# jhamrick/bayesian-quadrature

Measured on AMD Instinct MI355X. Metric: bq_fit_posterior_throughput, higher is better.
Workload: dtype f64; 1 GPU; C2: d=1 N=1024 M=256 Gaussian integrand, w=dx, s=1e-3; curve_workload=C5 shard: 64 x (d=1 N=2048 M=256), w=dx, s=1e-2, on_curve=True, bordered_system=1344

## Files before the change

bayesian-quadrature_amd/_lib.py:

```python
import ctypes as C
import os

import numpy as np

_HERE = os.path.dirname(os.path.abspath(__file__))
LIB_PATH = os.environ.get("BQHIP_LIBRARY") or os.path.join(_HERE, "libbqhip.so")
PROBE_LIB_PATH = os.environ.get("BQHIP_PROBE_LIBRARY") or \
    os.path.splitext(LIB_PATH)[0] + "_probe.so"

BQ_OK, BQ_ERR_NOT_PD, BQ_ERR_BAD_ARG, BQ_ERR_HIP, BQ_ERR_NOMEM = 0, 1, 2, 3, 4
BQ_MAX_DIM = 8
K_CLASSES = ("gram", "potf2", "trsm", "gemm_panel", "syrk_trailing", "syrk_trailing_small",
             "reduce")

_dp = C.POINTER(C.c_double)
_i32p = C.POINTER(C.c_int32)
_i64p = C.POINTER(C.c_int64)
_vp = C.c_void_p
_i64 = C.c_int64
_dbl = C.c_double

SIGNATURES = {
    "bq_device_count": (C.c_int, [C.POINTER(C.c_int)]),
    "bq_ctx_create": (C.c_int, [C.c_int, C.POINTER(_vp)]),
# ... 76 lines not shown
PROBE_SIGNATURES = {
    "bq_probe_xcd_hop": (C.c_int, [_vp, C.c_int, C.c_int64, C.c_int64, C.POINTER(C.c_double), _i32p,
                                   C.POINTER(C.c_int64)]),
    "bq_probe_mfma_f64": (C.c_int, [_vp, _dp]),
    "bq_probe_fma_f64": (C.c_int, [_vp, _dp]),
    "bq_probe_hbm": (C.c_int, [_vp, C.c_size_t, _dp, _dp]),
    "bq_probe_hbm_read8": (C.c_int, [_vp, C.c_size_t, _i64, _dp]),
    "bq_probe_gemm": (C.c_int, [_vp, _i64, _i64, _i64, C.c_int, _i64, C.c_int, _i64, _dp]),
    "bq_probe_gemm_product": (C.c_int, [_vp, _dp, _i64, _dp, _i64, _dp, _i64, _i64, _i64, _i64,
                                        C.c_int, _i64, C.c_int, _i64, C.c_int, C.c_int, _i64, C.c_int,
                                        C.c_int, _dp, _i32p, _i32p]),
    "bq_probe_mfma_variant": (C.c_int, [_vp, C.c_int, C.c_int, C.c_int, _dp]),
    "bq_probe_mfma444_layout": (C.c_int, [_vp, C.c_int, C.c_int, _i32p]),
    "bq_probe_launch": (C.c_int, [_vp, _i64, _dp]),
    "bq_probe_c2_timeline": (C.c_int, [_vp, _vp, C.POINTER(C.c_int64), _i64]),
    "bq_probe_exp": (C.c_int, [_vp, _dp, _i64, _dp]),
    "bq_probe_potf2": (C.c_int, [_vp, _dp, C.c_int, _i64, _dp, _dp, C.POINTER(C.c_int32), _dp,
                                 C.POINTER(C.c_int64)]),
    "bq_probe_mfma_layout": (C.c_int, [_vp, _dp]),
    "bq_probe_panel_solve": (C.c_int, [_vp, _i64, _i64, _i64, _dp, _dp, C.c_int, _i64, _dp]),
    "bq_probe_potrf_batch": (C.c_int, [_vp, _i64, _i64, _i64, _i64, _i64, _dp, _i32p, _i32p]),
    "bq_probe_sweep": (C.c_int, [_vp, C.c_int, _i64, _dp, _i64, _i64, _i64, _dp, _i32p]),
}

_lib = None
_probe_lib = None


class LibraryMissing(ImportError):
    pass
# ... 46 lines not shown
```

bayesian-quadrature_amd/csrc/ctx.hip:

```cpp
#include "host.h"

namespace bqh {

int prof_collect(bq_ctx *c)
{
    if (c->prof_events.empty())
        return BQ_OK;
    HIPCHK(c, hipStreamSynchronize(c->stream));
    if (c->aux)
        HIPCHK(c, hipStreamSynchronize(c->aux));
    if (c->prof_keep_timeline && !c->prof_origin)
        c->prof_origin = c->prof_events.front().a;
    for (auto &e : c->prof_events) {
        float ms = 0.f;
        if (hipEventElapsedTime(&ms, e.a, e.b) == hipSuccess) {
            c->prof_ms[e.cls] += ms;
            c->prof_n[e.cls] += 1;
            c->prof_work[e.cls] += e.work;
            if (c->prof_keep_timeline) {
                float t0 = 0.f;
                (void)hipEventElapsedTime(&t0, c->prof_origin, e.a);
                c->prof_timeline.insert(c->prof_timeline.end(),
                                        {(double)e.cls, (double)e.on_aux, (double)t0,
                                         (double)t0 + ms, e.work});
// ... 79 lines not shown
        {"BQ_TRSV_FLOW", &bq_ctx::trsv_flow},
        {"BQ_LOOKAHEAD", &bq_ctx::lookahead},
        {"BQ_DIAG_FIRST", &bq_ctx::diag_first},
        {"BQ_ASM_FUSE", &bq_ctx::asm_fuse},
        {"BQ_DF_SWEEP", &bq_ctx::df_sweep},
        {"BQ_DF_WG", &bq_ctx::df_wg},
        {"BQ_PAIR_BORDER", &bq_ctx::pair_border},
        {"BQ_DF_WG_ROWS", &bq_ctx::df_wg_rows},
        {"BQ_DF_EARLY", &bq_ctx::df_early},
        {"BQ_SOLVE_KCOPY", &bq_ctx::solve_kcopy},
        {"BQ_LA_MIN", &bq_ctx::la_min},
        {"BQ_GEMM_LDS", &bq_ctx::gemm_lds},
        {"BQ_FOLD_READOUT", &bq_ctx::fold_readout},
        {"BQ_POTF2_8W", &bq_ctx::potf2_8w},
        {"BQ_SLAB8_ROUNDS", &bq_ctx::slab8_rounds},
        {"BQ_GEMM_KSPLIT", &bq_ctx::gemm_ksplit},
        {"BQ_GEMM_TILE", &bq_ctx::gemm_tile},
        {"BQ_GRAPH", &bq_ctx::use_graph},
    };
    for (const auto &sw : switches)
        if (const char *e = std::getenv(sw.name))
            c->*sw.field = std::atoi(e);
    return BQ_OK;
}

extern "C" int bq_ctx_create(int device, bq_ctx **out)
{
    if (!out)
        return BQ_ERR_BAD_ARG;
    *out = nullptr;
// ... 288 lines not shown
```

bayesian-quadrature_amd/csrc/gram.h:

```cpp
#pragma once
#include "common.h"
#include "seed.h"

template <int D>
__global__ __launch_bounds__(256) void gram_sym_kernel(const double *__restrict__ x, long xstride,
                                                       const GaussParams *__restrict__ gp,
                                                       int gpstride, double *__restrict__ K,
                                                       long ldk, long kstride, int n)
{
    const int b = blockIdx.z;
    x += (long)b * xstride;
    K += (long)b * kstride;
    const GaussParams g = gp[(long)b * gpstride];
    const int t = threadIdx.x;
    const int i = blockIdx.x * 128 + (t & 63) * 2;
    const int jbase = blockIdx.y * 64 + (t >> 6) * 16;
    if (i >= n)
        return;
    const bool two = (i + 1 < n);
    double xi0[D], xi1[D];
#pragma unroll
    for (int k = 0; k < D; ++k) {
        xi0[k] = x[k + (long)i * D];
        xi1[k] = two ? x[k + (long)(i + 1) * D] : 0.0;
// ... 124 lines not shown
            const int j = min(jbase + h8 + jj, n2 - 1);
#pragma unroll
            for (int k = 0; k < D; ++k)
                xj[jj][k] = x2[k + (long)j * D];
        }
#pragma unroll
        for (int jj = 0; jj < 8; ++jj) {
            const int j = jbase + h8 + jj;
            const double e = g.c * exp_gauss(gauss_q<D>(xi, xj[jj], g));
            K[i + (long)j * ldk] = (row && j < n2) ? e : 0.0;
        }
    }
}


template <int D>
__device__ __forceinline__ void assemble_tile(const double *__restrict__ pts,
                                              const double *__restrict__ y, const GaussParams &g,
                                              double *__restrict__ A, long lda, const Layout &L,
                                              double *__restrict__ S0, long lds, int ib = -1,
                                              int jb = -1, int ilim = 0x7fffffff,
                                              int jlim = 0x7fffffff)
{
    const int t = threadIdx.x;
    if (ib < 0) {
        ib = blockIdx.x * 128;
        jb = blockIdx.y * 64;
    }
    if (jb > ib + 127)
        return;
    const int i = ib + (t & 63) * 2;
    const int jbase = jb + (t >> 6) * 16;
    if (i >= L.ntot || i >= ilim)
        return;
    bool pi[2];
    double xi[2][D];
#pragma unroll
    for (int r = 0; r < 2; ++r) {
        const int ii = i + r;
        pi[r] = (ii < L.n) || (ii >= L.npad && ii < L.npad + L.M);
#pragma unroll
        for (int k = 0; k < D; ++k)
            xi[r][k] = pi[r] ? pts[k + (long)ii * D] : 0.0;
    }
    for (int jj = 0; jj < 16; ++jj) {
        const int j = jbase + jj;
        if (j >= L.ntot || j >= jlim)
            break;
        const bool pj = (j < L.n) || (j >= L.npad && j < L.npad + L.M);
        double xj[D];
#pragma unroll
        for (int k = 0; k < D; ++k)
            xj[k] = pj ? pts[k + (long)j * D] : 0.0;
        double v[2];
#pragma unroll
        for (int r = 0; r < 2; ++r)
            v[r] = bordered_entry<D>(i + r, j, pi[r], pj, xi[r], xj, g, L, y);
        double2_t vv = {v[0], v[1]};
        *reinterpret_cast<double2_t *>(A + i + (long)j * lda) = vv;
        if (S0 && jb == 0 && i >= 64)
            *reinterpret_cast<double2_t *>(S0 + i + (long)j * lds) = vv;
    }
}

template <int D>
__global__ __launch_bounds__(256) void assemble_kernel(const double *__restrict__ pts,
                                                       long pstride, const double *__restrict__ y,
                                                       long ystride,
                                                       const GaussParams *__restrict__ gp,
                                                       int gpstride, double *__restrict__ A,
                                                       long lda, long astride, Layout L)
{
    const int b = blockIdx.z;
    assemble_tile<D>(pts + (long)b * pstride, y + (long)b * ystride, gp[(long)b * gpstride],
                     A + (long)b * astride, lda, L, nullptr, 0);
}

template <int D>
__global__ __launch_bounds__(256) void assemble_region_kernel(const double *__restrict__ pts,
                                                              long pstride,
                                                              const double *__restrict__ y,
                                                              long ystride,
                                                              const GaussParams *__restrict__ gp,
                                                              int gpstride, double *__restrict__ A,
                                                              long lda, long astride, Layout L, int r,
                                                              int c, int m, int n)
{
    const int b = blockIdx.z;
    assemble_tile<D>(pts + (long)b * pstride, y + (long)b * ystride, gp[(long)b * gpstride],
                     A + (long)b * astride, lda, L, nullptr, 0, r + (int)blockIdx.x * 128,
                     c + (int)blockIdx.y * 64, r + m, c + n);
}
```

bayesian-quadrature_amd/csrc/host.h:

```cpp
#pragma once
#include <hip/hip_runtime.h>

#pragma GCC visibility push(default)
#include "../../include/bqhip.h"
#pragma GCC visibility pop

#include "types.h"

#include <algorithm>
#include <cmath>
#include <cstdarg>
#include <cstdio>
#include <cstdlib>
#include <cstring>
#include <limits>
#include <new>
#include <string>
#include <vector>

#define BQ_GUARD_BYTES 4096
inline bool &devbuf_guard()
{
    static bool on = std::getenv("BQ_GUARD") && std::atoi(std::getenv("BQ_GUARD"));
    return on;
// ... 77 lines not shown
    int *flow_abort = nullptr;
    long n_flow_fallback = 0;
    int pair_border = 1;
    int df_wg_rows = 1000;
    int df_early = 1;
    int solve_kcopy = 1;
    double *hstage = nullptr;
    size_t hstage_len = 0;
    int la_min = 3072;
    DevBuf panel_ws;
    DevBuf scratch;
    int gemm_lds = 1;
    int fold_readout = 1;
    int asm_fuse = 1;
    int potf2_8w = 1;
    int slab8_rounds = 1 << 20;
    int gemm_ksplit = 1;
    int gemm_tile = 0;
    int sharing = 0;
    int use_graph = 1;
    bool own_stream = false;
    int cus = 256;
    int nb_override = 0;
    bq_plan *plan_cache = nullptr;
    char err[512] = {0};
    hipEvent_t t0 = nullptr, t1 = nullptr;
    bool prof = false;
    std::vector<ProfEvent> prof_events;
    bool prof_keep_timeline = false;
    hipEvent_t prof_origin = nullptr;
// ... 31 lines not shown
    } while (0)

#define BQCHK(call)                                                                            \
    do {                                                                                       \
        int s__ = (call);                                                                      \
        if (s__ != BQ_OK)                                                                      \
            return s__;                                                                        \
    } while (0)

inline long roundup(long v, long q) { return (v + q - 1) / q * q; }

inline unsigned long long launch_config_key(const bq_ctx *c)
{
    const int f[] = {c->nb_override, c->lookahead, c->la_min,   c->gemm_lds,  c->fold_readout,
                     c->potf2_8w,    c->gemm_ksplit, c->gemm_tile, c->diag_first, c->df_sweep,
                     c->df_wg,       c->df_early,   c->df_wg_rows, c->slab8_rounds};
    unsigned long long h = 1469598103934665603ull;
    for (int v : f)
        h = (h ^ (unsigned long long)(unsigned)v) * 1099511628211ull;
    return h;
}

inline long pick_ld(long ntot)
{
    long ld = ntot;
    if (ntot >= 1024 && (ntot % 512) == 0)
        ld += 64;
    return ld;
}

inline GaussParams make_params(int d, double h, const double *w, double s)
// ... 74 lines not shown
int check_w(bq_ctx *c, int64_t d, double h, const double *w, double s);

int launch_gram_sym(bq_ctx *c, int d, const double *x, long xstride, const GaussParams *gp,
                    int gpstride, double *K, long ldk, long kstride, int n, int batch);
int launch_gram_cross(bq_ctx *c, int d, const double *x1, int n1, const double *x2, int n2,
                      const GaussParams &g, double *K, long ldk);
int launch_gram_cross_pad(bq_ctx *c, int d, const double *x1, int n1, int n1p, const double *x2,
                          int n2, int n2p, const GaussParams &g, double *K, long ldk);

struct FirstStep {
    double *S0 = nullptr;
    long lds = 0, sstride = 0;
    double *dinv = nullptr;
    int *info = nullptr;
    double *scal = nullptr;
};
int launch_assemble(bq_ctx *c, int d, const double *pts, long pstride, const double *y,
                    long ystride, const GaussParams *gp, int gpstride, double *A, long lda,
                    long astride, Layout L, int batch, const FirstStep &fs = FirstStep(),
                    int jcols = 0);
int launch_assemble_region(bq_ctx *c, const GramSeed &sd, double *A, long lda, long astride, int m,
                           int n, int batch);
int launch_potf2(bq_ctx *c, double *A, long lda, long astride, int j0, double *dinv, long dstride,
                 int *info, int batch);
int launch_potrf_wg(bq_ctx *c, double *A, long lda, long astride, int kb, double *rec, long rstride,
                    int *info, int col0, int batch);
int launch_trsm_blk(bq_ctx *c, double *X, long ldx, long xstride, int m, const double *L11,
                    long ldl, long lstride, const double *dinv, long dstride, int batch);
int launch_diag_winv(bq_ctx *c, const double *L, long ldl, int npad, double *dw);
int launch_panel_step(bq_ctx *c, double *A, long lda, long astride, int batch, int nrb,
// ... 428 lines not shown
```

bayesian-quadrature_amd/csrc/k_panel.hip:

```cpp
#include "host.h"
#include "gram.h"
#include "trsm.h"
#include "slab.h"

namespace bqh {

template <int D>
void launch_assemble_d(bq_ctx *c, const double *pts, long pstride, const double *y, long ystride,
                       const GaussParams *gp, int gpstride, double *A, long lda, long astride,
                       Layout L, int batch, const FirstStep &fs, int jcols)
{
    dim3 grid((L.ntot + 127) / 128, ((jcols > 0 ? jcols : L.ntot) + 63) / 64, batch);
    const long wgs = (long)grid.x * grid.y * grid.z;
    if (fs.S0 && c->potf2_8w && wgs <= 2L * c->cus)
        hipLaunchKernelGGL((assemble_first_kernel<D, 8>), grid, dim3(512), 0, c->cur, pts, pstride, y,
                           ystride, gp, gpstride, A, lda, astride, L, fs.S0, fs.lds, fs.sstride,
                           fs.dinv, (long)BQ_DINV_STRIDE, fs.info, fs.scal);
    else if (fs.S0)
        hipLaunchKernelGGL((assemble_first_kernel<D, 4>), grid, dim3(256), 0, c->cur, pts, pstride, y,
                           ystride, gp, gpstride, A, lda, astride, L, fs.S0, fs.lds, fs.sstride,
                           fs.dinv, (long)BQ_DINV_STRIDE, fs.info, fs.scal);
    else
        hipLaunchKernelGGL(assemble_kernel<D>, grid, dim3(256), 0, c->cur, pts, pstride, y, ystride,
                           gp, gpstride, A, lda, astride, L);
}

int launch_assemble(bq_ctx *c, int d, const double *pts, long pstride, const double *y,
                    long ystride, const GaussParams *gp, int gpstride, double *A, long lda,
                    long astride, Layout L, int batch, const FirstStep &fs, int jcols)
{
    if (jcols < 0 || (jcols & 63) || jcols > L.ntot || (jcols > 0 && fs.S0))
        return fail(c, BQ_ERR_BAD_ARG, "assemble: column limit");
    const double cols = jcols > 0 ? jcols : L.ntot;
    Bracket br(c, BQ_K_GRAM, 8.0 * cols * (L.ntot - 0.5 * cols + 0.5) * batch);
    switch (d) {
    case 1: launch_assemble_d<1>(c, pts, pstride, y, ystride, gp, gpstride, A, lda, astride, L, batch, fs, jcols); break;
    case 2: launch_assemble_d<2>(c, pts, pstride, y, ystride, gp, gpstride, A, lda, astride, L, batch, fs, jcols); break;
    case 3: launch_assemble_d<3>(c, pts, pstride, y, ystride, gp, gpstride, A, lda, astride, L, batch, fs, jcols); break;
    case 4: launch_assemble_d<4>(c, pts, pstride, y, ystride, gp, gpstride, A, lda, astride, L, batch, fs, jcols); break;
    case 5: launch_assemble_d<5>(c, pts, pstride, y, ystride, gp, gpstride, A, lda, astride, L, batch, fs, jcols); break;
    case 6: launch_assemble_d<6>(c, pts, pstride, y, ystride, gp, gpstride, A, lda, astride, L, batch, fs, jcols); break;
    case 7: launch_assemble_d<7>(c, pts, pstride, y, ystride, gp, gpstride, A, lda, astride, L, batch, fs, jcols); break;
    case 8: launch_assemble_d<8>(c, pts, pstride, y, ystride, gp, gpstride, A, lda, astride, L, batch, fs, jcols); break;
    default: return fail(c, BQ_ERR_BAD_ARG, "d must be in 1..%d", BQ_MAXD);
    }
    HIPCHK(c, hipGetLastError());
    return BQ_OK;
// ... 144 lines not shown
```

bayesian-quadrature_amd/csrc/potf2.h:

```cpp
#pragma once
#include "common.h"

template <int NW> struct Potf2FT {
    double a[16 / NW][4];
};
using Potf2F = Potf2FT<4>;

#define BQ_POTF2F_SLOTS (16 * 256)
#define BQ_POTF2F_LDS_DOUBLES (BQ_POTF2F_SLOTS + 1024)

template <int P, int NW = 4>
__device__ __forceinline__ void potf2f_factor(Potf2FT<NW> &st, double *slot, int lane)
{
    constexpr int QP = P / NW;
    double dn = st.a[QP][0];
#pragma unroll
    for (int s = 0; s < 4; ++s) {
        const int c = 4 * P + s;
        const double d = readlane_f64(dn, c);
        const double y0 = __builtin_amdgcn_rsq(d);
        const double t = d * y0;
        const double l0 = st.a[QP][s] * y0;
        const double e = __builtin_fma(-t, y0, 1.0);
        const double p = __builtin_fma(0.375, e, 0.5);
// ... 188 lines not shown
struct Potf2FSteps<16, NW, PAD, EARLY> {
    static __device__ __forceinline__ void run(Potf2FT<NW> &, double *, int, int, long long *, int)
    {
    }
};

#define BQ_STAMP(k)                                                                                \
    if (stamps && threadIdx.x == 0)                                                                \
    stamps[k] = (long long)__builtin_amdgcn_s_memtime()

template <int NW = 4>
__device__ __forceinline__ void potf2f_run(Potf2FT<NW> &st, double *__restrict__ Ab, long lda,
                                           int j0, double *__restrict__ dinv_b,
                                           int *__restrict__ info_b, double *lds,
                                           long long *stamps = nullptr, double *logdet = nullptr,
                                           int nreal = 64)
{
    constexpr int NG = 16 / NW;
    const int lane = threadIdx.x & 63;
    const int w = __builtin_amdgcn_readfirstlane(threadIdx.x >> 6);
    double *slots = lds;
    double *blk = lds + BQ_POTF2F_SLOTS;
    BQ_STAMP(1);
    if (w == 0)
        potf2f_factor<0, NW>(st, slots, lane);
    if (nreal >= 64) {
        const double ld0 = logdet ? *logdet : 0.0;
        Potf2FSteps<0, NW, false, true>::run(
            st, slots, w, lane,
            (stamps && stamps[5] != 0) ? stamps + 8 : nullptr, 64);
        BQ_STAMP(2);
        BQ_STAMP(3);
        if (NW == 8 && w >= 4) {
            const int c0 = 16 * (w - 4);
            double *pw = Ab + lane + (long)c0 * lda;
            const double *ps = slots + 64 * c0 + lane;
            asm volatile("" : "+v"(pw));
            double col[16];
#pragma unroll
            for (int c = 0; c < 16; ++c)
                col[c] = ps[64 * c];
#pragma unroll
// ... 8 lines not shown
            for (int q = 0; q < NG; ++q) {
#pragma unroll
                for (int s = 0; s < 4; ++s)
                    if (lane >= 4 * (NW * q + w) + s)
                        pw[(long)s * lda] = st.a[q][s];
                pw += 4 * NW * lda;
            }
        }
        constexpr int WR = NW == 8 ? 4 : 1, WL = NW == 8 ? 5 : 2;
        if (w < 4)
            potf2f_inverse(slots, w, dinv_b + 64 + 256 * w, lane);
        if (w == WR) {
            const double dg = slots[256 * (lane >> 2) + 64 * (lane & 3) + lane];
            dinv_b[lane] = potf2f_rcp(dg);
            const unsigned long long badm = __ballot(!(dg > 0.0) || !(dg < 1.7e308));
            if (lane == 0 && badm != 0ull && info_b[0] == 0)
                info_b[0] = j0 + __builtin_ctzll(badm) + 1;
        }
        if (w == WL && logdet) {
            const double lg = potf2f_wave_sum(log(slots[256 * (lane >> 2) + 64 * (lane & 3) + lane]));
            if (lane == 0)
                *logdet = ld0 + 2.0 * lg;
        }
        BQ_STAMP(4);
        return;
    }
    Potf2FSteps<0, NW, true>::run(st, slots, w, lane, nullptr, nreal > 0 ? nreal : 1);
    BQ_STAMP(2);
    {
        const int bq = lane >> 4, i16 = lane & 15;
#pragma unroll
// ... 12 lines not shown
        asm volatile("" : "+v"(pw));
#pragma unroll
        for (int q = 0; q < NG; ++q) {
#pragma unroll
            for (int s = 0; s < 4; ++s)
                if (lane >= 4 * (NW * q + w) + s)
                    pw[(long)s * lda] = st.a[q][s];
            pw += 4 * NW * lda;
        }
    }
#define BQ_POTF2F_LOGDET                                                                           \
    {                                                                                              \
        double lg = log(blk[256 * (lane >> 4) + 17 * (lane & 15)]);                                \
        _Pragma("unroll") for (int off = 32; off > 0; off >>= 1) lg += __shfl_down(lg, off, 64);   \
        if (lane == 0)                                                                             \
            *logdet += 2.0 * lg;                                                                   \
    }
    if (NW > 4 && w >= 4) {
        if (logdet && w == 4)
            BQ_POTF2F_LOGDET
        return;
    }
    {
        const double dg = blk[256 * (lane >> 4) + 17 * (lane & 15)];
        double rc = __builtin_amdgcn_rcp(dg);
        rc = __builtin_fma(__builtin_fma(-dg, rc, 1.0), rc, rc);
        rc = __builtin_fma(__builtin_fma(-dg, rc, 1.0), rc, rc);
        if (w == 0) {
            dinv_b[lane] = rc;
            const unsigned long long badm = __ballot(!(dg > 0.0) || !(dg < 1.7e308));
            if (lane == 0 && badm != 0ull && info_b[0] == 0)
                info_b[0] = j0 + __builtin_ctzll(badm) + 1;
        }
        const double *bw = blk + 256 * w;
        double sv[16], wc[16];
#pragma unroll
        for (int i = 0; i < 16; ++i)
            sv[i] = (i == (lane & 15)) ? 1.0 : 0.0;
        double cur[16], nxt[16];
#pragma unroll
        for (int i = 1; i < 16; ++i)
            cur[i] = bw[i];
#pragma unroll
        for (int k = 0; k < 16; ++k) {
            if (k < 14) {
#pragma unroll
// ... 63 lines not shown
```

bayesian-quadrature_amd/csrc/probe.hip:

```cpp
#include "host.h"

#pragma GCC visibility push(default)
#include "../../include/bqhip_probe.h"
#pragma GCC visibility pop

#include "probe.h"

using namespace bqh;

extern "C" int bq_probe_mfma_f64(bq_ctx *c, double *tflops)
{
    if (!c || !tflops)
        return BQ_ERR_BAD_ARG;
    HIPCHK(c, hipSetDevice(c->device));
    DevBuf o;
    HIPCHK(c, o.alloc(64));
    const int iters = 4096, blocks = c->cus * 8;
    hipLaunchKernelGGL(probe_mfma_kernel, dim3(blocks), dim3(256), 0, c->stream, o.d(), 64);
    HIPCHK(c, hipStreamSynchronize(c->stream));
    float ms = 0;
    BQCHK(bq_timer_start(c));
    hipLaunchKernelGGL(probe_mfma_kernel, dim3(blocks), dim3(256), 0, c->stream, o.d(), iters);
    BQCHK(bq_timer_stop_ms(c, &ms));
    const double flops = (double)blocks * 4  * iters * 4  * (16.0 * 16 * 4 * 2);
// ... 610 lines not shown
                ran.B = 64;
                kind = BQ_SWEEP_KIND_BLK;
            }
        }
        HIPCHK(c, hipMemcpyAsync(X, res, xbytes, hipMemcpyDeviceToHost, c->stream));
        HIPCHK(c, hipStreamSynchronize(c->stream));
    }
    route[0] = kind;
    route[1] = ran.B;
    route[2] = ran.n_lds;
    route[3] = ran.n_splitk;
    route[4] = (int32_t)c->n_flow_fallback;
    return BQ_OK;
}

extern "C" int bq_probe_c2_timeline(bq_ctx *c, bq_plan *p, int64_t *stamps, int64_t nsteps)
{
    if (!c || !p || !stamps || nsteps < 1 || nsteps > 1024)
        return BQ_ERR_BAD_ARG;
    if (sweep_route(c, p->L.ntot, p->L.npad, p->nprob, p->panel.bytes / sizeof(double)).kind !=
        SweepRoute::Slab)
        return fail(c, BQ_ERR_BAD_ARG, "timeline: this plan does not sweep with the one-launch steps");
    if (nsteps < p->L.npad / 64)
        return fail(c, BQ_ERR_BAD_ARG, "timeline: %d steps, room for %d", p->L.npad / 64, (int)nsteps);
    HIPCHK(c, hipSetDevice(c->device));
    DevBuf st;
    HIPCHK(c, st.alloc(sizeof(long long) * 160 * (size_t)nsteps));
    HIPCHK(c, hipMemsetAsync(st.p, 0, st.bytes, c->stream));
    BQCHK(plan_enqueue(c, p, static_cast<long long *>(st.p), (int)nsteps));
    HIPCHK(c, hipMemcpyAsync(stamps, st.p, st.bytes, hipMemcpyDeviceToHost, c->stream));
// ... 4 lines not shown
```

bayesian-quadrature_amd/csrc/seed.h:

```cpp
#pragma once
#include "common.h"

template <int D>
__device__ __forceinline__ double bordered_entry(int ii, int j, bool pi, bool pj,
                                                 const double (&xi)[D], const double (&xj)[D],
                                                 const GaussParams &g, const Layout &L,
                                                 const double *__restrict__ y)
{
    if (pi && pj) {
        double val = g.c * exp_gauss(gauss_q<D>(xi, xj, g));
        if (ii == j && ii < L.n)
            val += g.s2;
        return val;
    }
    if (ii == L.yrow)
        return (j < L.n) ? y[j] : 0.0;
    return (ii == j) ? 1.0 : 0.0;
}

template <int D, int TM, int TN>
__device__ __forceinline__ void gram_seed_neg(double (&acc)[TM][TN][4], const GramSeed &sd, int b,
                                              int row0, int col0, int lane)
{
    const int l15 = lane & 15, l4 = lane >> 4, blk = (lane >> 2) & 3;
    const double *__restrict__ pts = sd.pts + (long)b * sd.pstride;
    const double *__restrict__ y = sd.y + (long)b * sd.ystride;
    const GaussParams g = sd.gp[(long)b * sd.gpstride];
    const Layout L = sd.L;
    bool pi[TM];
    double xi[TM][D];
#pragma unroll
    for (int tm = 0; tm < TM; ++tm) {
// ... 24 lines not shown
```

bayesian-quadrature_amd/csrc/slab.h:

```cpp
#pragma once
#include "common.h"
#include "potf2.h"


__device__ __forceinline__ void slab_load16(const double *__restrict__ S, long lds,
                                            double (&t)[4][4])
{
#pragma unroll
    for (int c = 0; c < 4; ++c)
#pragma unroll
        for (int r = 0; r < 4; ++r)
            t[c][r] = S[(long)(16 * c + 4 * r) * lds];
}

__device__ __forceinline__ void slab_solve16(const double (&t)[4][4], const double (&la)[4][3][4],
                                             const double (&wneg)[4][4], double4_t (&x)[4])
{
#pragma unroll
    for (int c = 0; c < 4; ++c) {
        double4_t acc = {-t[c][0], -t[c][1], -t[c][2], -t[c][3]};
#pragma unroll
        for (int bb = 0; bb < c; ++bb)
#pragma unroll
            for (int r = 0; r < 4; ++r)
// ... 313 lines not shown
#pragma unroll
            for (int r = 0; r < 4; ++r)
                Cout[(long)(16 * cb + 4 * r) * ldo] = -acc[cb][r];
        if (emit) {
#pragma unroll
            for (int cb = 0; cb < 4; ++cb)
#pragma unroll
                for (int r = 0; r < 4; ++r)
                    BQ_SLAB_EMIT(Rb + 16 * wave + l15, Cb + 16 * cb + l4 + 4 * r, -acc[cb][r])
        }
    }
#undef BQ_SLAB_EMIT
#undef BQ_SSTAMP
}

template <int D, int NW = 4>
__global__ __launch_bounds__(64 * NW) void assemble_first_kernel(
    const double *__restrict__ pts, long pstride, const double *__restrict__ y, long ystride,
    const GaussParams *__restrict__ gp, int gpstride, double *__restrict__ A, long lda,
    long astride, Layout L, double *__restrict__ S0, long lds, long sstride,
    double *__restrict__ dinv, long dstride, int *__restrict__ info, double *__restrict__ scal)
{
    __shared__ __attribute__((aligned(16))) double plds[BQ_POTF2_LDS_DOUBLES];
    const int b = blockIdx.z;
    A += (long)b * astride;
    if (NW == 4 || threadIdx.x < 256)
        assemble_tile<D>(pts + (long)b * pstride, y + (long)b * ystride, gp[(long)b * gpstride],
                         A, lda, L, S0 + (long)b * sstride, lds);
    if (blockIdx.x == 0 && blockIdx.y == 0) {
        if (threadIdx.x == 0) {
            info[b] = 0;
            if (scal)
                scal[4 * b + 1] = 0.0;
        }
        asm volatile("s_waitcnt vmcnt(0)" ::: "memory");
        __syncthreads();
        __builtin_amdgcn_s_setprio(3);
        potf2_body<NW>(A, lda, 0, dinv + (long)b * dstride, info + b, plds, nullptr, 0, nullptr,
                       scal ? scal + 4 * b + 1 : nullptr, L.n);
    }
}

__global__ __launch_bounds__(256) void slab_first_kernel(double *__restrict__ A, long lda,
                                                         long astride, double *__restrict__ S,
                                                         long lds, long sstride, int ntot,
                                                         double *__restrict__ dinv, long dstride,
                                                         int *__restrict__ info, int col0)
{
    __shared__ __attribute__((aligned(16))) double plds[BQ_POTF2_LDS_DOUBLES];
    const int b = blockIdx.z;
    A += (long)b * astride;
    if (blockIdx.x == 0) {
        __builtin_amdgcn_s_setprio(3);
        potf2_body(A, lda, col0, dinv + (long)b * dstride, info + b, plds);
// ... 313 lines not shown
```

bayesian-quadrature_amd/engine.py:

```python
import ctypes as C

import numpy as np

from . import _lib as L

_dp = L._dp


def _pts(x):
    x = np.asarray(x, dtype=np.float64)
    if x.ndim == 1:
        x = x[None, :]
    if x.ndim != 2:
        raise ValueError("points must be a vector or a d x n matrix")
    return np.asfortranarray(x)


def _wvec(w, d):
    w = np.atleast_1d(np.asarray(w, dtype=np.float64)).ravel().copy()
    if w.shape[0] != d:
        raise ValueError("w has invalid shape")
    return w


# ... 452 lines not shown
        e = self.probe_engine()
        if buf.dtype != np.float64 or buf.ndim != 1 or not buf.flags.c_contiguous:
            raise ValueError("buf must be a flat contiguous float64 array")
        ld = int(lda) if lda else self.plan_ld(ntot)
        stride = int(astride) if astride else ld * int(ntot)
        if buf.shape[0] != stride * int(batch):
            raise ValueError("buf holds %d doubles, the batch %d" % (buf.shape[0], stride * batch))
        info = np.full(int(batch), -1, dtype=np.int32)
        route = np.full(3, -1, dtype=np.int32)
        e._check(e._lib.bq_probe_potrf_batch(
            e._ctx, int(batch), int(ntot), int(ntot if ncols is None else ncols), int(lda),
            int(astride), L.dptr(buf), info.ctypes.data_as(L._i32p),
            route.ctypes.data_as(L._i32p)))
        return info, (self.SWEEP_KINDS[route[0]], int(route[1]), bool(route[2]))

    SWEEPS = ("forward_rows", "backward_rows", "forward_rows_blk", "inverse_rows", "forward_vec",
              "backward_vec", "forward_vec_flow", "backward_vec_flow")
    ROWS_KINDS = ("step", "fused", "gemm_rows", "blk", "vec_block", "vec_flow")

    def probe_sweep(self, which, Lfac, X, mrows=None, ldl=0):
        e = self.probe_engine()
        Lf = L.f64(Lfac)
        n = Lf.shape[0]
        if Lf.shape != (n, n):
            raise ValueError("Lfac must be square")
        if X.dtype != np.float64 or X.ndim != 2 or not X.flags.f_contiguous or X.shape[1] != n:
            raise ValueError("X must be a Fortran-ordered float64 (ldx, n) array")
        ldx = X.shape[0]
        route = np.full(5, -1, dtype=np.int32)
        e._check(e._lib.bq_probe_sweep(
# ... 344 lines not shown
```

include/bqhip_probe.h:

```cpp
#ifndef BQHIP_PROBE_H
#define BQHIP_PROBE_H

#include "bqhip.h"

#ifdef __cplusplus
extern "C" {
#endif

int bq_probe_mfma_f64(bq_ctx *ctx, double *tflops);
int bq_probe_fma_f64(bq_ctx *ctx, double *tflops);
int bq_probe_hbm(bq_ctx *ctx, size_t bytes, double *write_gbs, double *copy_gbs);
int bq_probe_xcd_hop(bq_ctx *ctx, int mode, int64_t iters, int64_t kib, double *ns_per_hop,
                     int32_t *xcc16, int64_t *bad_words);
int bq_probe_gemm(bq_ctx *ctx, int64_t m, int64_t n, int64_t k, int lower, int64_t batch, int qt,
                  int64_t reps, double *ms);
int bq_probe_gemm_product(bq_ctx *ctx, double *C, int64_t ldc, const double *P, int64_t ldp,
                          const double *Q, int64_t ldq, int64_t m, int64_t n, int64_t k, int lower,
                          int64_t batch, int qt, int64_t ccut, int sharing, int want_fuse, int64_t j0,
                          int seed_d, int rows, double *dinv, int32_t *info, int32_t *route);
int bq_probe_hbm_read8(bq_ctx *ctx, size_t bytes, int64_t reps, double *read_gbs);
int bq_probe_mfma_variant(bq_ctx *ctx, int kind, int nacc, int blocks_per_cu, double *tflops);
int bq_probe_mfma444_layout(bq_ctx *ctx, int cbsz, int abid, int32_t *out8192);
int bq_probe_exp(bq_ctx *ctx, const double *x, int64_t n, double *out);
int bq_probe_launch(bq_ctx *ctx, int64_t n, double *us_per_launch);
int bq_probe_c2_timeline(bq_ctx *ctx, bq_plan *plan, int64_t *stamps, int64_t nsteps);
int bq_probe_potf2(bq_ctx *ctx, const double *A, int from_lds, int64_t reps, double *L_out,
                   double *dinv_out, int32_t *info_out, double *us_per_launch,
                   int64_t *stamps136);
int bq_probe_panel_solve(bq_ctx *ctx, int64_t m, int64_t kb, int64_t batch, const double *L,
                         double *X, int mode, int64_t reps, double *ms_per_call);
int bq_probe_potrf_batch(bq_ctx *ctx, int64_t batch, int64_t ntot, int64_t ncols, int64_t lda,
                         int64_t astride, double *A, int32_t *info, int32_t *route);
enum {
    BQ_SWEEP_FORWARD_ROWS = 0,
    BQ_SWEEP_BACKWARD_ROWS = 1,
    BQ_SWEEP_FORWARD_ROWS_BLK = 2,
    BQ_SWEEP_INVERSE_ROWS = 3,
    BQ_SWEEP_FORWARD_VEC = 4,
    BQ_SWEEP_BACKWARD_VEC = 5,
    BQ_SWEEP_FORWARD_VEC_FLOW = 6,
// ... 19 lines not shown
```

Measured before the change: 4188 problems/s.

## Factor the first diagonal block from registers inside the assembly launch

The first assembly launch now has the corner workgroup compute the 64x64 diagonal block straight into the potf2 register tile and factor it immediately. It no longer waits for all tiles to be stored and reloaded. A separate workgroup assembles the rest of that first tile column, so the grid is widened to at least three column blocks. The general tile assembly is also restructured to preload column points and y values in batches and to use a flattened, branch-free entry evaluation. It also adds a 'fresh' mode so info and logdet are initialised inside potf2 rather than by a separate store, plus a timestamped probe entry point. The risk is higher register pressure and extra workgroups in the launch.

```diff
diff --git a/bayesian-quadrature_amd/_lib.py b/bayesian-quadrature_amd/_lib.py
--- a/bayesian-quadrature_amd/_lib.py
+++ b/bayesian-quadrature_amd/_lib.py
@@ -114,6 +114,9 @@
     "bq_probe_mfma444_layout": (C.c_int, [_vp, C.c_int, C.c_int, _i32p]),
     "bq_probe_launch": (C.c_int, [_vp, _i64, _dp]),
     "bq_probe_c2_timeline": (C.c_int, [_vp, _vp, C.POINTER(C.c_int64), _i64]),
+    "bq_probe_first_launch": (C.c_int, [_vp, _i64, _i64, _i64, _i64, _dp, _dp, _dp, C.c_double, _dp,
+                                        C.c_double, _i64, _i64, _dp, _dp, _dp, _i32p, _dp,
+                                        C.POINTER(C.c_int64)]),
     "bq_probe_exp": (C.c_int, [_vp, _dp, _i64, _dp]),
     "bq_probe_potf2": (C.c_int, [_vp, _dp, C.c_int, _i64, _dp, _dp, C.POINTER(C.c_int32), _dp,
                                  C.POINTER(C.c_int64)]),
diff --git a/bayesian-quadrature_amd/csrc/ctx.hip b/bayesian-quadrature_amd/csrc/ctx.hip
--- a/bayesian-quadrature_amd/csrc/ctx.hip
+++ b/bayesian-quadrature_amd/csrc/ctx.hip
@@ -117,6 +117,7 @@
         {"BQ_FOLD_READOUT", &bq_ctx::fold_readout},
         {"BQ_POTF2_8W", &bq_ctx::potf2_8w},
         {"BQ_SLAB8_ROUNDS", &bq_ctx::slab8_rounds},
+        {"BQ_FIRST_REGS", &bq_ctx::first_regs},
         {"BQ_GEMM_KSPLIT", &bq_ctx::gemm_ksplit},
         {"BQ_GEMM_TILE", &bq_ctx::gemm_tile},
         {"BQ_GRAPH", &bq_ctx::use_graph},
diff --git a/bayesian-quadrature_amd/csrc/gram.h b/bayesian-quadrature_amd/csrc/gram.h
--- a/bayesian-quadrature_amd/csrc/gram.h
+++ b/bayesian-quadrature_amd/csrc/gram.h
@@ -162,9 +162,12 @@
 }
 
 
-template <int D>
+#ifndef BQ_ASM_TILE_CB
+#define BQ_ASM_TILE_CB 4
+#endif
+template <int D, int CBW = 0>
 __device__ __forceinline__ void assemble_tile(const double *__restrict__ pts,
-                                              const double *__restrict__ y, const GaussParams &g,
+                                              const double *__restrict__ y, const GaussParams &gm,
                                               double *__restrict__ A, long lda, const Layout &L,
                                               double *__restrict__ S0, long lds, int ib = -1,
                                               int jb = -1, int ilim = 0x7fffffff,
@@ -179,35 +182,68 @@
         return;
     const int i = ib + (t & 63) * 2;
     const int jbase = jb + (t >> 6) * 16;
-    if (i >= L.ntot || i >= ilim)
-        return;
+    if (i >= L.ntot || i >= ilim || jbase >= L.ntot || jbase >= jlim)
+        return;
+    GaussParams g;
+    g.c = gm.c, g.s2 = gm.s2;
+#pragma unroll
+    for (int k = 0; k < D; ++k)
+        g.nh[k] = gm.nh[k];
     bool pi[2];
     double xi[2][D];
 #pragma unroll
     for (int r = 0; r < 2; ++r) {
         const int ii = i + r;
         pi[r] = (ii < L.n) || (ii >= L.npad && ii < L.npad + L.M);
+        const long ic = pi[r] ? ii : 0;
 #pragma unroll
         for (int k = 0; k < D; ++k)
-            xi[r][k] = pi[r] ? pts[k + (long)ii * D] : 0.0;
-    }
-    for (int jj = 0; jj < 16; ++jj) {
-        const int j = jbase + jj;
-        if (j >= L.ntot || j >= jlim)
-            break;
-        const bool pj = (j < L.n) || (j >= L.npad && j < L.npad + L.M);
-        double xj[D];
-#pragma unroll
-        for (int k = 0; k < D; ++k)
-            xj[k] = pj ? pts[k + (long)j * D] : 0.0;
-        double v[2];
-#pragma unroll
-        for (int r = 0; r < 2; ++r)
-            v[r] = bordered_entry<D>(i + r, j, pi[r], pj, xi[r], xj, g, L, y);
-        double2_t vv = {v[0], v[1]};
-        *reinterpret_cast<double2_t *>(A + i + (long)j * lda) = vv;
-        if (S0 && jb == 0 && i >= 64)
-            *reinterpret_cast<double2_t *>(S0 + i + (long)j * lds) = vv;
+            xi[r][k] = pts[k + ic * D];
+    }
+    const bool yt = L.yrow >= ib && L.yrow < ib + 128;
+    const double *__restrict__ ysrc = yt ? y : pts;
+    const bool to_s0 = S0 && jb == 0 && i >= 64;
+    constexpr int CBMAX = D == 1 ? 16 : (D == 2 ? 8 : 4);
+    constexpr int CB = CBW > 0 && CBW < CBMAX ? CBW : CBMAX;
+    constexpr int LB = (CBW == 0 && D <= 2) ? 16 : CB;
+#pragma unroll
+    for (int l0 = 0; l0 < 16; l0 += LB) {
+        bool pj[LB];
+        double xj[LB][D], yj[LB];
+#pragma unroll
+        for (int jj = 0; jj < LB; ++jj) {
+            const int j = jbase + l0 + jj;
+            pj[jj] = (j < L.n) || (j >= L.npad && j < L.npad + L.M);
+            const long jc = pj[jj] ? j : 0;
+#pragma unroll
+            for (int k = 0; k < D; ++k)
+                xj[jj][k] = pts[k + jc * D];
+            yj[jj] = ysrc[j < L.n ? j : 0];
+        }
+        __builtin_amdgcn_sched_barrier(0);
+#pragma unroll
+        for (int c0 = 0; c0 < LB; c0 += CB) {
+            const int j0 = l0 + c0;
+            double2_t vv[CB];
+#pragma unroll
+            for (int jj = 0; jj < CB; ++jj) {
+                const int j = jbase + j0 + jj;
+#pragma unroll
+                for (int r = 0; r < 2; ++r)
+                    vv[jj][r] = bordered_entry_flat<D>(i + r, j, pi[r], pj[c0 + jj], xi[r],
+                                                       xj[c0 + jj], g, L, yj[c0 + jj]);
+            }
+#pragma unroll
+            for (int jj = 0; jj < CB; ++jj)
+                *reinterpret_cast<double2_t *>(A + i + (long)(jbase + j0 + jj) * lda) = vv[jj];
+            if (to_s0) {
+#pragma unroll
+                for (int jj = 0; jj < CB; ++jj)
+                    *reinterpret_cast<double2_t *>(S0 + i + (long)(jbase + j0 + jj) * lds) = vv[jj];
+            }
+            if (CB < LB)
+                __builtin_amdgcn_sched_barrier(0);
+        }
     }
 }
 
@@ -220,7 +256,7 @@
                                                        long lda, long astride, Layout L)
 {
     const int b = blockIdx.z;
-    assemble_tile<D>(pts + (long)b * pstride, y + (long)b * ystride, gp[(long)b * gpstride],
+    assemble_tile<D, BQ_ASM_TILE_CB>(pts + (long)b * pstride, y + (long)b * ystride, gp[(long)b * gpstride],
                      A + (long)b * astride, lda, L, nullptr, 0);
 }
 
@@ -235,7 +271,7 @@
                                                               int c, int m, int n)
 {
     const int b = blockIdx.z;
-    assemble_tile<D>(pts + (long)b * pstride, y + (long)b * ystride, gp[(long)b * gpstride],
+    assemble_tile<D, BQ_ASM_TILE_CB>(pts + (long)b * pstride, y + (long)b * ystride, gp[(long)b * gpstride],
                      A + (long)b * astride, lda, L, nullptr, 0, r + (int)blockIdx.x * 128,
                      c + (int)blockIdx.y * 64, r + m, c + n);
 }
diff --git a/bayesian-quadrature_amd/csrc/host.h b/bayesian-quadrature_amd/csrc/host.h
--- a/bayesian-quadrature_amd/csrc/host.h
+++ b/bayesian-quadrature_amd/csrc/host.h
@@ -115,6 +115,7 @@
     int fold_readout = 1;
     int asm_fuse = 1;
     int potf2_8w = 1;
+    int first_regs = 1;
     int slab8_rounds = 1 << 20;
     int gemm_ksplit = 1;
     int gemm_tile = 0;
@@ -176,7 +177,8 @@
 {
     const int f[] = {c->nb_override, c->lookahead, c->la_min,   c->gemm_lds,  c->fold_readout,
                      c->potf2_8w,    c->gemm_ksplit, c->gemm_tile, c->diag_first, c->df_sweep,
-                     c->df_wg,       c->df_early,   c->df_wg_rows, c->slab8_rounds};
+                     c->df_wg,       c->df_early,   c->df_wg_rows, c->slab8_rounds,
+                     c->first_regs};
     unsigned long long h = 1469598103934665603ull;
     for (int v : f)
         h = (h ^ (unsigned long long)(unsigned)v) * 1099511628211ull;
@@ -281,6 +283,7 @@
     double *dinv = nullptr;
     int *info = nullptr;
     double *scal = nullptr;
+    long long *stamps = nullptr;
 };
 int launch_assemble(bq_ctx *c, int d, const double *pts, long pstride, const double *y,
                     long ystride, const GaussParams *gp, int gpstride, double *A, long lda,
diff --git a/bayesian-quadrature_amd/csrc/k_panel.hip b/bayesian-quadrature_amd/csrc/k_panel.hip
--- a/bayesian-quadrature_amd/csrc/k_panel.hip
+++ b/bayesian-quadrature_amd/csrc/k_panel.hip
@@ -11,18 +11,43 @@
                        Layout L, int batch, const FirstStep &fs, int jcols)
 {
     dim3 grid((L.ntot + 127) / 128, ((jcols > 0 ? jcols : L.ntot) + 63) / 64, batch);
-    const long wgs = (long)grid.x * grid.y * grid.z;
-    if (fs.S0 && c->potf2_8w && wgs <= 2L * c->cus)
-        hipLaunchKernelGGL((assemble_first_kernel<D, 8>), grid, dim3(512), 0, c->cur, pts, pstride, y,
-                           ystride, gp, gpstride, A, lda, astride, L, fs.S0, fs.lds, fs.sstride,
-                           fs.dinv, (long)BQ_DINV_STRIDE, fs.info, fs.scal);
-    else if (fs.S0)
-        hipLaunchKernelGGL((assemble_first_kernel<D, 4>), grid, dim3(256), 0, c->cur, pts, pstride, y,
-                           ystride, gp, gpstride, A, lda, astride, L, fs.S0, fs.lds, fs.sstride,
-                           fs.dinv, (long)BQ_DINV_STRIDE, fs.info, fs.scal);
-    else
+    if (!fs.S0) {
         hipLaunchKernelGGL(assemble_kernel<D>, grid, dim3(256), 0, c->cur, pts, pstride, y, ystride,
                            gp, gpstride, A, lda, astride, L);
+        return;
+    }
+    const bool regs = c->first_regs != 0;
+    if (regs && grid.y < 3)
+        grid.y = 3;
+    const long wgs = (long)grid.x * grid.y * grid.z;
+    const bool w8 = c->potf2_8w && wgs <= 2L * c->cus;
+#define BQ_ASM_FIRST(NW_, REGS_, STAMP_)                                                           \
+    hipLaunchKernelGGL((assemble_first_kernel<D, NW_, REGS_, STAMP_>), grid, dim3(64 * NW_), 0,    \
+                       c->cur, pts, pstride, y, ystride, gp, gpstride, A, lda, astride, L, fs.S0,  \
+                       fs.lds, fs.sstride, fs.dinv, (long)BQ_DINV_STRIDE, fs.info, fs.scal,        \
+                       fs.stamps)
+    if constexpr (D == 1) {
+        if (fs.stamps) {
+            if (w8 && regs)
+                BQ_ASM_FIRST(8, true, true);
+            else if (w8)
+                BQ_ASM_FIRST(8, false, true);
+            else if (regs)
+                BQ_ASM_FIRST(4, true, true);
+            else
+                BQ_ASM_FIRST(4, false, true);
+            return;
+        }
+    }
+    if (w8 && regs)
+        BQ_ASM_FIRST(8, true, false);
+    else if (w8)
+        BQ_ASM_FIRST(8, false, false);
+    else if (regs)
+        BQ_ASM_FIRST(4, true, false);
+    else
+        BQ_ASM_FIRST(4, false, false);
+#undef BQ_ASM_FIRST
 }
 
 int launch_assemble(bq_ctx *c, int d, const double *pts, long pstride, const double *y,
@@ -31,6 +56,8 @@
 {
     if (jcols < 0 || (jcols & 63) || jcols > L.ntot || (jcols > 0 && fs.S0))
         return fail(c, BQ_ERR_BAD_ARG, "assemble: column limit");
+    if (fs.stamps && (!fs.S0 || d != 1))
+        return fail(c, BQ_ERR_BAD_ARG, "assemble: the stamped first launch is one-dimensional");
     const double cols = jcols > 0 ? jcols : L.ntot;
     Bracket br(c, BQ_K_GRAM, 8.0 * cols * (L.ntot - 0.5 * cols + 0.5) * batch);
     switch (d) {
diff --git a/bayesian-quadrature_amd/csrc/potf2.h b/bayesian-quadrature_amd/csrc/potf2.h
--- a/bayesian-quadrature_amd/csrc/potf2.h
+++ b/bayesian-quadrature_amd/csrc/potf2.h
@@ -226,7 +226,7 @@
                                            int j0, double *__restrict__ dinv_b,
                                            int *__restrict__ info_b, double *lds,
                                            long long *stamps = nullptr, double *logdet = nullptr,
-                                           int nreal = 64)
+                                           int nreal = 64, bool fresh = false)
 {
     constexpr int NG = 16 / NW;
     const int lane = threadIdx.x & 63;
@@ -237,7 +237,7 @@
     if (w == 0)
         potf2f_factor<0, NW>(st, slots, lane);
     if (nreal >= 64) {
-        const double ld0 = logdet ? *logdet : 0.0;
+        const double ld0 = (logdet && !fresh) ? *logdet : 0.0;
         Potf2FSteps<0, NW, false, true>::run(
             st, slots, w, lane,
             (stamps && stamps[5] != 0) ? stamps + 8 : nullptr, 64);
@@ -276,7 +276,9 @@
             const double dg = slots[256 * (lane >> 2) + 64 * (lane & 3) + lane];
             dinv_b[lane] = potf2f_rcp(dg);
             const unsigned long long badm = __ballot(!(dg > 0.0) || !(dg < 1.7e308));
-            if (lane == 0 && badm != 0ull && info_b[0] == 0)
+            if (lane == 0 && fresh)
+                info_b[0] = badm != 0ull ? j0 + __builtin_ctzll(badm) + 1 : 0;
+            else if (lane == 0 && badm != 0ull && info_b[0] == 0)
                 info_b[0] = j0 + __builtin_ctzll(badm) + 1;
         }
         if (w == WL && logdet) {
@@ -319,7 +321,7 @@
         double lg = log(blk[256 * (lane >> 4) + 17 * (lane & 15)]);                                \
         _Pragma("unroll") for (int off = 32; off > 0; off >>= 1) lg += __shfl_down(lg, off, 64);   \
         if (lane == 0)                                                                             \
-            *logdet += 2.0 * lg;                                                                   \
+            *logdet = (fresh ? 0.0 : *logdet) + 2.0 * lg;                                          \
     }
     if (NW > 4 && w >= 4) {
         if (logdet && w == 4)
@@ -334,7 +336,9 @@
         if (w == 0) {
             dinv_b[lane] = rc;
             const unsigned long long badm = __ballot(!(dg > 0.0) || !(dg < 1.7e308));
-            if (lane == 0 && badm != 0ull && info_b[0] == 0)
+            if (lane == 0 && fresh)
+                info_b[0] = badm != 0ull ? j0 + __builtin_ctzll(badm) + 1 : 0;
+            else if (lane == 0 && badm != 0ull && info_b[0] == 0)
                 info_b[0] = j0 + __builtin_ctzll(badm) + 1;
         }
         const double *bw = blk + 256 * w;
diff --git a/bayesian-quadrature_amd/csrc/probe.hip b/bayesian-quadrature_amd/csrc/probe.hip
--- a/bayesian-quadrature_amd/csrc/probe.hip
+++ b/bayesian-quadrature_amd/csrc/probe.hip
@@ -648,6 +648,77 @@
     return BQ_OK;
 }
 
+extern "C" int bq_probe_first_launch(bq_ctx *c, int64_t batch, int64_t d, int64_t n, int64_t M,
+                                     const double *x, const double *y, const double *xo, double h,
+                                     const double *w, double s, int64_t ntot, int64_t dinv_len,
+                                     double *Acol, double *S0, double *dinv, int32_t *info,
+                                     double *scal, int64_t *stamps16)
+{
+    if (!c)
+        return BQ_ERR_BAD_ARG;
+    BQCHK(check_dims(c, d, n));
+    if (batch < 1 || batch > 65535 || M < 0 || M > 4096 || !x || !y || (!xo && M) || !w || !Acol ||
+        !S0 || !dinv || !info || !scal)
+        return fail(c, BQ_ERR_BAD_ARG, "first_launch: illegal value");
+    BQCHK(check_w(c, d, h, w, s));
+    const Layout L = make_layout((int)n, (int)M, true);
+    const long lda = pick_ld(L.ntot), astride = lda * (long)L.ntot;
+    if (ntot != L.ntot || dinv_len != BQ_DINV_STRIDE)
+        return fail(c, BQ_ERR_BAD_ARG, "first_launch: buffers for ntot = %d and %d doubles of record, not %lld and %lld",
+                    L.ntot, (int)BQ_DINV_STRIDE, (long long)ntot, (long long)dinv_len);
+    if (!sweep_route(c, L.ntot, L.npad, (int)batch, ~(size_t)0 >> 1).first_in_assembly)
+        return fail(c, BQ_ERR_BAD_ARG, "first_launch: this shape's sweep has no first launch in the assembly");
+    HIPCHK(c, hipSetDevice(c->device));
+    DevBuf A, pts, yd, gp, dv, ws, inf, sc, st;
+    HIPCHK(c, A.alloc(sizeof(double) * (size_t)astride * batch));
+    HIPCHK(c, pts.alloc(sizeof(double) * (size_t)d * L.ntot * batch));
+    HIPCHK(c, yd.alloc(sizeof(double) * (size_t)L.npad * batch));
+    HIPCHK(c, gp.alloc(sizeof(GaussParams) * (size_t)batch));
+    HIPCHK(c, dv.alloc(sizeof(double) * BQ_DINV_STRIDE * (size_t)batch));
+    HIPCHK(c, ws.alloc(sizeof(double) * 64 * (size_t)L.ntot * batch));
+    HIPCHK(c, inf.alloc(sizeof(int) * (size_t)batch));
+    HIPCHK(c, sc.alloc(sizeof(double) * 4 * (size_t)batch));
+    HIPCHK(c, st.alloc(sizeof(long long) * 16));
+    for (DevBuf *b : {&A, &dv, &ws, &inf, &sc})
+        HIPCHK(c, hipMemsetAsync(b->p, 0xA5, b->bytes, c->stream));
+    HIPCHK(c, hipMemsetAsync(pts.p, 0, pts.bytes, c->stream));
+    HIPCHK(c, hipMemsetAsync(yd.p, 0, yd.bytes, c->stream));
+    HIPCHK(c, hipMemsetAsync(st.p, 0, st.bytes, c->stream));
+    std::vector<GaussParams> hgp((size_t)batch, make_params((int)d, h, w, s));
+    HIPCHK(c, hipMemcpyAsync(gp.p, hgp.data(), gp.bytes, hipMemcpyHostToDevice, c->stream));
+    HIPCHK(c, hipMemcpy2DAsync(pts.p, sizeof(double) * d * L.ntot, x, sizeof(double) * d * n,
+                               sizeof(double) * d * n, batch, hipMemcpyHostToDevice, c->stream));
+    if (M > 0)
+        HIPCHK(c, hipMemcpy2DAsync(pts.d() + (size_t)d * L.npad, sizeof(double) * d * L.ntot, xo,
+                                   sizeof(double) * d * M, sizeof(double) * d * M, batch,
+                                   hipMemcpyHostToDevice, c->stream));
+    HIPCHK(c, hipMemcpy2DAsync(yd.p, sizeof(double) * L.npad, y, sizeof(double) * n,
+                               sizeof(double) * n, batch, hipMemcpyHostToDevice, c->stream));
+    FirstStep fs;
+    fs.S0 = ws.d();
+    fs.lds = L.ntot;
+    fs.sstride = 64L * L.ntot;
+    fs.dinv = dv.d();
+    fs.info = inf.i();
+    fs.scal = sc.d();
+    fs.stamps = stamps16 ? static_cast<long long *>(st.p) : nullptr;
+    BQCHK(launch_assemble(c, (int)d, pts.d(), (long)d * L.ntot, yd.d(), L.npad,
+                          static_cast<const GaussParams *>(gp.p), 1, A.d(), lda, astride, L,
+                          (int)batch, fs));
+    for (int64_t b = 0; b < batch; ++b)
+        HIPCHK(c, hipMemcpy2DAsync(Acol + (size_t)b * 64 * L.ntot, sizeof(double) * L.ntot,
+                                   A.d() + (size_t)b * astride, sizeof(double) * lda,
+                                   sizeof(double) * L.ntot, 64, hipMemcpyDeviceToHost, c->stream));
+    HIPCHK(c, hipMemcpyAsync(S0, ws.p, ws.bytes, hipMemcpyDeviceToHost, c->stream));
+    HIPCHK(c, hipMemcpyAsync(dinv, dv.p, dv.bytes, hipMemcpyDeviceToHost, c->stream));
+    HIPCHK(c, hipMemcpyAsync(info, inf.p, inf.bytes, hipMemcpyDeviceToHost, c->stream));
+    HIPCHK(c, hipMemcpyAsync(scal, sc.p, sc.bytes, hipMemcpyDeviceToHost, c->stream));
+    if (stamps16)
+        HIPCHK(c, hipMemcpyAsync(stamps16, st.p, st.bytes, hipMemcpyDeviceToHost, c->stream));
+    HIPCHK(c, hipStreamSynchronize(c->stream));
+    return BQ_OK;
+}
+
 extern "C" int bq_probe_c2_timeline(bq_ctx *c, bq_plan *p, int64_t *stamps, int64_t nsteps)
 {
     if (!c || !p || !stamps || nsteps < 1 || nsteps > 1024)
diff --git a/bayesian-quadrature_amd/csrc/seed.h b/bayesian-quadrature_amd/csrc/seed.h
--- a/bayesian-quadrature_amd/csrc/seed.h
+++ b/bayesian-quadrature_amd/csrc/seed.h
@@ -1,11 +1,15 @@
 #pragma once
 #include "common.h"
 
-template <int D>
-__device__ __forceinline__ double bordered_entry(int ii, int j, bool pi, bool pj,
-                                                 const double (&xi)[D], const double (&xj)[D],
-                                                 const GaussParams &g, const Layout &L,
-                                                 const double *__restrict__ y)
+struct YHeld {
+    double v;
+    __device__ __forceinline__ double operator[](int) const { return v; }
+};
+
+template <int D, class Y>
+__device__ __forceinline__ double bordered_entry_y(int ii, int j, bool pi, bool pj,
+                                                   const double (&xi)[D], const double (&xj)[D],
+                                                   const GaussParams &g, const Layout &L, Y y)
 {
     if (pi && pj) {
         double val = g.c * exp_gauss(gauss_q<D>(xi, xj, g));
@@ -16,6 +20,26 @@
     if (ii == L.yrow)
         return (j < L.n) ? y[j] : 0.0;
     return (ii == j) ? 1.0 : 0.0;
+}
+
+template <int D>
+__device__ __forceinline__ double bordered_entry(int ii, int j, bool pi, bool pj,
+                                                 const double (&xi)[D], const double (&xj)[D],
+                                                 const GaussParams &g, const Layout &L,
+                                                 const double *__restrict__ y)
+{
+    return bordered_entry_y<D, const double *__restrict__>(ii, j, pi, pj, xi, xj, g, L, y);
+}
+
+template <int D>
+__device__ __forceinline__ double bordered_entry_flat(int ii, int j, bool pi, bool pj,
+                                                      const double (&xi)[D], const double (&xj)[D],
+                                                      const GaussParams &g, const Layout &L,
+                                                      double yj)
+{
+    const double kv = bordered_entry_y<D, YHeld>(ii, j, true, true, xi, xj, g, L, YHeld{yj});
+    const double ov = bordered_entry_y<D, YHeld>(ii, j, false, false, xi, xj, g, L, YHeld{yj});
+    return (pi && pj) ? kv : ov;
 }
 
 template <int D, int TM, int TN>
diff --git a/bayesian-quadrature_amd/csrc/slab.h b/bayesian-quadrature_amd/csrc/slab.h
--- a/bayesian-quadrature_amd/csrc/slab.h
+++ b/bayesian-quadrature_amd/csrc/slab.h
@@ -351,20 +351,106 @@
 #undef BQ_SSTAMP
 }
 
-template <int D, int NW = 4>
+
+template <int D, int NW>
+__device__ __forceinline__ void first_block_regs(Potf2FT<NW> &st, const double *__restrict__ pts,
+                                                 const GaussParams &gm, double *__restrict__ A,
+                                                 long lda, const Layout &L, int wv, int lane)
+{
+    constexpr int NG = 16 / NW;
+    constexpr int GQ = 4 * NG * D <= 32 ? NG : 1;
+    Layout L0 = L;
+    L0.yrow = -1;
+    GaussParams g;
+    g.c = gm.c, g.s2 = gm.s2;
+#pragma unroll
+    for (int k = 0; k < D; ++k)
+        g.nh[k] = gm.nh[k];
+    const bool pi = lane < L.n;
+    double xi[D];
+#pragma unroll
+    for (int k = 0; k < D; ++k)
+        xi[k] = pts[k + (long)(pi ? lane : 0) * D];
+#pragma unroll
+    for (int q0 = 0; q0 < NG; q0 += GQ) {
+        double xj[GQ][4][D];
+#pragma unroll
+        for (int q = 0; q < GQ; ++q)
+#pragma unroll
+            for (int s = 0; s < 4; ++s) {
+                const int c = 4 * (NW * (q0 + q) + wv) + s;
+#pragma unroll
+                for (int k = 0; k < D; ++k)
+                    xj[q][s][k] = pts[k + (long)(c < L.n ? c : 0) * D];
+            }
+        __builtin_amdgcn_sched_barrier(0);
+#pragma unroll
+        for (int q = 0; q < GQ; ++q)
+#pragma unroll
+            for (int s = 0; s < 4; ++s) {
+                const int c = 4 * (NW * (q0 + q) + wv) + s;
+                st.a[q0 + q][s] =
+                    bordered_entry_flat<D>(lane, c, pi, c < L.n, xi, xj[q][s], g, L0, 0.0);
+            }
+    }
+#pragma unroll
+    for (int q = 0; q < NG; ++q)
+#pragma unroll
+        for (int s = 0; s < 4; ++s)
+            PIN(st.a[q][s]);
+#pragma unroll
+    for (int q = 0; q < NG; ++q)
+#pragma unroll
+        for (int s = 0; s < 4; ++s) {
+            const int c = 4 * (NW * q + wv) + s;
+            if (lane < c)
+                A[lane + (long)c * lda] = st.a[q][s];
+        }
+}
+
+template <int D, int NW = 4, bool REGS = true, bool STAMP = false>
 __global__ __launch_bounds__(64 * NW) void assemble_first_kernel(
     const double *__restrict__ pts, long pstride, const double *__restrict__ y, long ystride,
     const GaussParams *__restrict__ gp, int gpstride, double *__restrict__ A, long lda,
     long astride, Layout L, double *__restrict__ S0, long lds, long sstride,
-    double *__restrict__ dinv, long dstride, int *__restrict__ info, double *__restrict__ scal)
+    double *__restrict__ dinv, long dstride, int *__restrict__ info, double *__restrict__ scal,
+    long long *stamps)
 {
     __shared__ __attribute__((aligned(16))) double plds[BQ_POTF2_LDS_DOUBLES];
     const int b = blockIdx.z;
+    const bool corner = blockIdx.x == 0 && blockIdx.y == 0;
+    long long *const st0 = (STAMP && corner && b == 0) ? stamps : nullptr;
+    if (st0 && threadIdx.x == 0)
+        st0[0] = (long long)__builtin_amdgcn_s_memtime();
     A += (long)b * astride;
+    if constexpr (REGS) {
+        if (blockIdx.x == 0 && blockIdx.y == 2) {
+            if (NW == 4 || threadIdx.x < 256)
+                assemble_tile<D>(pts + (long)b * pstride, y + (long)b * ystride,
+                                 gp[(long)b * gpstride], A, lda, L, S0 + (long)b * sstride, lds, 64,
+                                 0, 128);
+            return;
+        }
+        if (corner) {
+            __builtin_amdgcn_s_setprio(3);
+            const int lane = threadIdx.x & 63;
+            Potf2FT<NW> st;
+            first_block_regs<D, NW>(st, pts + (long)b * pstride, gp[(long)b * gpstride], A, lda, L,
+                                    (int)(threadIdx.x >> 6), lane);
+            if (st0) {
+                asm volatile("" ::"v"(st.a[0][0]));
+                if (threadIdx.x == 0)
+                    st0[1] = st0[2] = (long long)__builtin_amdgcn_s_memtime();
+            }
+            potf2f_run<NW>(st, A, lda, 0, dinv + (long)b * dstride, info + b, plds,
+                           st0 ? st0 + 2 : nullptr, scal ? scal + 4 * b + 1 : nullptr, L.n, true);
+            return;
+        }
+    }
     if (NW == 4 || threadIdx.x < 256)
         assemble_tile<D>(pts + (long)b * pstride, y + (long)b * ystride, gp[(long)b * gpstride],
                          A, lda, L, S0 + (long)b * sstride, lds);
-    if (blockIdx.x == 0 && blockIdx.y == 0) {
+    if (!REGS && corner) {
         if (threadIdx.x == 0) {
             info[b] = 0;
             if (scal)
@@ -372,9 +458,11 @@
         }
         asm volatile("s_waitcnt vmcnt(0)" ::: "memory");
         __syncthreads();
+        if (st0 && threadIdx.x == 0)
+            st0[1] = (long long)__builtin_amdgcn_s_memtime();
         __builtin_amdgcn_s_setprio(3);
-        potf2_body<NW>(A, lda, 0, dinv + (long)b * dstride, info + b, plds, nullptr, 0, nullptr,
-                       scal ? scal + 4 * b + 1 : nullptr, L.n);
+        potf2_body<NW>(A, lda, 0, dinv + (long)b * dstride, info + b, plds, nullptr, 0,
+                       st0 ? st0 + 2 : nullptr, scal ? scal + 4 * b + 1 : nullptr, L.n);
     }
 }
 
diff --git a/bayesian-quadrature_amd/engine.py b/bayesian-quadrature_amd/engine.py
--- a/bayesian-quadrature_amd/engine.py
+++ b/bayesian-quadrature_amd/engine.py
@@ -490,6 +490,35 @@
             route.ctypes.data_as(L._i32p)))
         return info, (self.SWEEP_KINDS[route[0]], int(route[1]), bool(route[2]))
 
+    def probe_first_launch(self, x, y, xo, h, w, s, stamps=False):
+        e = self.probe_engine()
+        x = np.asarray(x, dtype=np.float64)
+        B, d, n = x.shape
+        xo = np.zeros((B, d, 0)) if xo is None else np.asarray(xo, dtype=np.float64)
+        M = xo.shape[2]
+        y = np.ascontiguousarray(y, dtype=np.float64)
+        if y.shape != (B, n) or xo.shape != (B, d, M):
+            raise ValueError("y must be (B, n) and xo (B, d, M)")
+        xf = np.ascontiguousarray(np.transpose(x, (0, 2, 1)))
+        xof = np.ascontiguousarray(np.transpose(xo, (0, 2, 1)))
+        wv = np.ascontiguousarray(np.broadcast_to(np.asarray(w, dtype=np.float64), (d,)))
+        ntot = -(-(-(-n // 64) * 64 + M + 1) // 64) * 64
+        rec = 2 * (64 + 4 * 256)
+        out = {"A": np.empty((B, 64, ntot)), "S0": np.empty((B, 64, ntot)),
+               "dinv": np.empty((B, rec)), "info": np.empty(B, dtype=np.int32),
+               "scal": np.empty((B, 4))}
+        st = np.zeros(16, dtype=np.int64) if stamps else None
+        e._check(e._lib.bq_probe_first_launch(
+            e._ctx, B, d, n, M, L.dptr(xf), L.dptr(y), L.dptr(xof) if M else None, float(h),
+            L.dptr(wv), float(s), ntot, rec, L.dptr(out["A"]), L.dptr(out["S0"]), L.dptr(out["dinv"]),
+            out["info"].ctypes.data_as(L._i32p), L.dptr(out["scal"]),
+            st.ctypes.data_as(C.POINTER(C.c_int64)) if stamps else None))
+        out["A"] = np.transpose(out["A"], (0, 2, 1))
+        out["S0"] = np.transpose(out["S0"], (0, 2, 1))
+        if stamps:
+            out["stamps"] = st
+        return out
+
     SWEEPS = ("forward_rows", "backward_rows", "forward_rows_blk", "inverse_rows", "forward_vec",
               "backward_vec", "forward_vec_flow", "backward_vec_flow")
     ROWS_KINDS = ("step", "fused", "gemm_rows", "blk", "vec_block", "vec_flow")
diff --git a/include/bqhip_probe.h b/include/bqhip_probe.h
--- a/include/bqhip_probe.h
+++ b/include/bqhip_probe.h
@@ -24,6 +24,10 @@
 int bq_probe_exp(bq_ctx *ctx, const double *x, int64_t n, double *out);
 int bq_probe_launch(bq_ctx *ctx, int64_t n, double *us_per_launch);
 int bq_probe_c2_timeline(bq_ctx *ctx, bq_plan *plan, int64_t *stamps, int64_t nsteps);
+int bq_probe_first_launch(bq_ctx *ctx, int64_t batch, int64_t d, int64_t n, int64_t M,
+                          const double *x, const double *y, const double *xo, double h,
+                          const double *w, double s, int64_t ntot, int64_t dinv_len, double *Acol,
+                          double *S0, double *dinv, int32_t *info, double *scal, int64_t *stamps16);
 int bq_probe_potf2(bq_ctx *ctx, const double *A, int from_lds, int64_t reps, double *L_out,
                    double *dinv_out, int32_t *info_out, double *us_per_launch,
                    int64_t *stamps136);
```

New measurement: 4262 problems/s (median of 6 runs). 1.02x the previous value.
